# delldu/TransMVSNet

Hardware: AMD Instinct MI355X
Metric: depth maps/sec @ DTU 864x1152 N=5 (48/32/8 hyp); Abs depth L1 vs ref (higher is better)
Workload: dtype f32; 1 GPU; DTU 864x1152, N=5 views, cascade 48/32/8, B=1, hot path from FeatureNet outputs (FMT+pathway+stage glue+cost volume+CostRegNet+softmax/WTA); global_batch=1, parallelism=replica1, launch=hip_graph replay

## Files before the change

### transmvsnet_amd/csrc/costreg.hip

```cpp
#include "common.h"

namespace tmvs {

typedef float floatx4 __attribute__((ext_vector_type(4)));

template <int N>
struct VecN;
template <>
struct VecN<4> {
  float v[4];
  __device__ __forceinline__ void load(const float* p) {
    const float4 t = *reinterpret_cast<const float4*>(p);
    v[0] = t.x;
    v[1] = t.y;
    v[2] = t.z;
    v[3] = t.w;
  }
  __device__ __forceinline__ void zero() { v[0] = v[1] = v[2] = v[3] = 0.f; }
};
template <>
struct VecN<2> {
  float v[2];
  __device__ __forceinline__ void load(const float* p) {
    const float2 t = *reinterpret_cast<const float2*>(p);
// ... 360 lines not shown
            for (int r = 0; r < NBW; ++r)
#pragma unroll
              for (int m = 0; m < MBW; ++m)
                acc[r][m] = __builtin_amdgcn_mfma_f32_16x16x4f32(a[m].v[j], b[r].v[j], acc[r][m], 0, 0, 0);
        }
      }
    }
  }
  if (ow >= g.Wo) return;
  const size_t out_n = (size_t)n * g.Do * g.Ho * g.Wo;
#pragma unroll
  for (int m = 0; m < MBW; ++m) {
    const int co = (mg * MBW + m) * 16 + kgrp * 4;
    if (co >= COUT) continue;
    const float4 al = *reinterpret_cast<const float4*>(alpha + co);
    const float4 sh = *reinterpret_cast<const float4*>(shift + co);
#pragma unroll
    for (int r = 0; r < NBW; ++r) {
      const int oh = hg * NBW + r;
      if (oh >= g.Ho) continue;
      float4 o;
      o.x = act(fmaf(acc[r][m][0], al.x, sh.x), g.lo);
      o.y = act(fmaf(acc[r][m][1], al.y, sh.y), g.lo);
      o.z = act(fmaf(acc[r][m][2], al.z, sh.z), g.lo);
      o.w = act(fmaf(acc[r][m][3], al.w, sh.w), g.lo);
      *reinterpret_cast<float4*>(y + (out_n + ((size_t)od * g.Ho + oh) * g.Wo + ow) * COUT + co) = o;
    }
  }
}

#ifndef TMVS_DECONV_ABL
#define TMVS_DECONV_ABL 0
#endif
template <int CIN, int COUT, int TDI, int THI, int MBB>
__global__ __launch_bounds__(256) void deconv3d_lds_kernel(const float* __restrict__ x,
                                                           const float* __restrict__ wpk,
                                                           const float* __restrict__ alpha,
                                                           const float* __restrict__ shift,
                                                           const float* __restrict__ skip, float* __restrict__ y,
                                                           Geo g) {
  constexpr int CK = CIN < 16 ? CIN : 16;
  constexpr int PL = CK / 4;
  constexpr int MB = (COUT + 15) / 16;
  constexpr int MG = MB / MBB;
  constexpr int NBW = TDI * THI / 4;
  constexpr int LW = 17, LH = THI + 1, LD = TDI + 1;
  constexpr bool SWZ = (CK == 16);
  constexpr int VST = SWZ ? 16 : CK + 4;
  constexpr int NVOX = LD * LH * LW;
  static_assert(MB % MBB == 0 && (TDI * THI) % 4 == 0, "tile");
  static_assert(CK == 16 && MBB == 1, "LDS weight staging assumes 16-channel chunks, one 16-row block");
  constexpr int RM = COUT < 16 ? COUT : 16;
  __shared__ __attribute__((aligned(16))) float tile[NVOX * VST];
  __shared__ __attribute__((aligned(16))) float wts[27 * RM * 16];

  const int nws = (g.Wi + 15) / 16, nhs = (g.Hi + THI - 1) / THI, nds = (g.Di + TDI - 1) / TDI;
  int t = xcd_remap(blockIdx.x, gridDim.x);
  const int mg = t % MG;
  t /= MG;
  const int ws = t % nws;
  t /= nws;
  const int hs = t % nhs;
  t /= nhs;
  const int ds = t % nds;
  const int n = t / nds;
  const int mw0 = ws * 16, mh0 = hs * THI, md0 = ds * TDI;
  const int lane = threadIdx.x & 63, wv = threadIdx.x >> 6;
  const int col = lane & 15, kgrp = lane >> 4;
  const size_t in_n = (size_t)n * g.Di * g.Hi * g.Wi;

  floatx4 acc[NBW][8][MBB];
#pragma unroll
  for (int r = 0; r < NBW; ++r)
#pragma unroll
    for (int c = 0; c < 8; ++c)
#pragma unroll
      for (int m = 0; m < MBB; ++m) acc[r][c][m] = floatx4{0.f, 0.f, 0.f, 0.f};

#pragma unroll 1
  for (int ch = 0; ch < CIN / CK; ++ch) {
    if (ch) __syncthreads();
    for (int idx = threadIdx.x; idx < ((TMVS_DECONV_ABL & 2) ? 0 : NVOX * PL); idx += 256) {
      const int vox = idx / PL, q = idx - vox * PL;
      const int lw = vox % LW, rest = vox / LW, lh = rest % LH, ld = rest / LH;
      const int iw = mw0 + lw, ih = mh0 + lh, id = md0 + ld;
      float4 v = make_float4(0.f, 0.f, 0.f, 0.f);
      if (iw < g.Wi && ih < g.Hi && id < g.Di)
        v = *reinterpret_cast<const float4*>(x + (in_n + ((size_t)id * g.Hi + ih) * g.Wi + iw) * CIN + ch * CK + 4 * q);
      const int qs = SWZ ? (q ^ ((vox >> 1) & 3)) : q;
      *reinterpret_cast<float4*>(tile + vox * VST + 4 * qs) = v;
    }
    for (int idx = threadIdx.x; idx < ((TMVS_DECONV_ABL & 1) ? 0 : 27 * RM * 4); idx += 256) {
      const int q = idx & 3, row = (idx >> 2) % RM, tap = (idx >> 2) / RM;
      const float4 v = *reinterpret_cast<const float4*>(wpk + ((size_t)tap * COUT + mg * 16 + row) * CIN + ch * CK + 4 * q);
      *reinterpret_cast<float4*>(wts + (tap * RM + row) * 16 + 4 * (q ^ ((row >> 1) & 3))) = v;
    }
    __syncthreads();
#pragma unroll
    for (int cls = 0; cls < 8; ++cls) {
      const int pd = cls >> 2, ph = (cls >> 1) & 1, pw = cls & 1;
#pragma unroll
      for (int td = 0; td < 1 + pd; ++td)
#pragma unroll
        for (int th = 0; th < 1 + ph; ++th)
#pragma unroll
          for (int tw = 0; tw < 1 + pw; ++tw) {
            const int kd = pd ? (td ? 2 : 0) : 1, od_off = (pd && !td) ? 1 : 0;
            const int kh = ph ? (th ? 2 : 0) : 1, oh_off = (ph && !th) ? 1 : 0;
            const int kw = pw ? (tw ? 2 : 0) : 1, ow_off = (pw && !tw) ? 1 : 0;
            const int tap = kd * 9 + kh * 3 + kw;
            VecN<PL> a[MBB];
            if (col < RM)
              a[0].load(wts + (tap * RM + col) * 16 + 4 * (kgrp ^ ((col >> 1) & 3)));
            else
              a[0].zero();
#pragma unroll
            for (int r = 0; r < NBW; ++r) {
              const int rr = wv * NBW + r;
              const int mdl = rr / THI, mhl = rr - mdl * THI;
              VecN<PL> b;
              const int lvox = ((mdl + od_off) * LH + mhl + oh_off) * LW + col + ow_off;
              const int qs = SWZ ? (kgrp ^ ((lvox >> 1) & 3)) : kgrp;
              b.load(tile + lvox * VST + qs * PL);
#pragma unroll
              for (int j = 0; j < PL; ++j)
#pragma unroll
                for (int m = 0; m < MBB; ++m) {
                  if (TMVS_DECONV_ABL & 4)
                    acc[r][cls][m][0] = fmaf(a[m].v[j], b.v[j], acc[r][cls][m][0]);
                  else
                    acc[r][cls][m] = __builtin_amdgcn_mfma_f32_16x16x4f32(a[m].v[j], b.v[j], acc[r][cls][m], 0, 0, 0);
                }
            }
          }
    }
  }
  const size_t out_n = (size_t)n * g.Do * g.Ho * g.Wo;
  if constexpr (COUT == 8) {
    __shared__ __attribute__((aligned(16))) float ep[4][32 * 8];
    float* eb = ep[wv];
    const int co = kgrp * 4;
    float4 al = make_float4(0.f, 0.f, 0.f, 0.f), sh = al;
    if (kgrp < 2) {
// ... 29 lines not shown
    }
    return;
  }
  const int mw = mw0 + col;
  if (mw >= g.Wi) return;
#pragma unroll
  for (int m = 0; m < MBB; ++m) {
    const int co = (mg * MBB + m) * 16 + kgrp * 4;
    if (co >= COUT) continue;
    const float4 al = *reinterpret_cast<const float4*>(alpha + co);
    const float4 sh = *reinterpret_cast<const float4*>(shift + co);
#pragma unroll
    for (int r = 0; r < NBW; ++r) {
      const int rr = wv * NBW + r;
      const int md = md0 + rr / THI, mh = mh0 + rr % THI;
      if (md >= g.Di || mh >= g.Hi) continue;
#pragma unroll
      for (int cls = 0; cls < 8; ++cls) {
        const int od = 2 * md + (cls >> 2), oh = 2 * mh + ((cls >> 1) & 1), ow = 2 * mw + (cls & 1);
        const size_t o = (out_n + ((size_t)od * g.Ho + oh) * g.Wo + ow) * COUT + co;
        const float4 s = skip ? *reinterpret_cast<const float4*>(skip + o) : make_float4(0.f, 0.f, 0.f, 0.f);
        float4 v;
        v.x = s.x + act(fmaf(acc[r][cls][m][0], al.x, sh.x), g.lo);
        v.y = s.y + act(fmaf(acc[r][cls][m][1], al.y, sh.y), g.lo);
        v.z = s.z + act(fmaf(acc[r][cls][m][2], al.z, sh.z), g.lo);
        v.w = s.w + act(fmaf(acc[r][cls][m][3], al.w, sh.w), g.lo);
        *reinterpret_cast<float4*>(y + o) = v;
      }
    }
  }
}

constexpr int kDChunk = 8;

constexpr int kProbCols = 62;
typedef float float2_v __attribute__((ext_vector_type(2)));

__device__ __forceinline__ float lane_from_left(float v) {
  return __int_as_float(__builtin_amdgcn_update_dpp(0, __float_as_int(v), 0x138, 0xF, 0xF, false));
}
__device__ __forceinline__ float lane_from_right(float v) {
  return __int_as_float(__builtin_amdgcn_update_dpp(0, __float_as_int(v), 0x130, 0xF, 0xF, false));
}

__global__ __launch_bounds__(256) void conv0_kernel(const float* __restrict__ x, float* __restrict__ y, int D, int H,
                                                    int W, const float* __restrict__ wt,
                                                    const float* __restrict__ alpha,
                                                    const float* __restrict__ shift, float lo) {
  const int HW = H * W;
  const int nseg = (W + kProbCols - 1) / kProbCols, nrow = (H + 3) / 4, ndc = (D + kDChunk - 1) / kDChunk;
  int lb = xcd_remap(blockIdx.x, gridDim.x);
  const int seg = lb % nseg;
  lb /= nseg;
  const int rowb = lb % nrow;
  lb /= nrow;
  const int dc = lb % ndc;
  const int n = lb / ndc;
  const int lane = threadIdx.x & 63;
  const int h = rowb * 4 + (threadIdx.x >> 6);
  if (h >= H) return;
  const int w = seg * kProbCols + lane - 1;
  const bool writes = lane >= 1 && lane <= kProbCols && w < W;
  const int d0 = dc * kDChunk, d1 = min(D, d0 + kDChunk);
  const __amdgpu_buffer_rsrc_t rx = raw_rsrc(x + (size_t)n * D * HW, (unsigned)(D * HW * 4));
  float* yp = y + ((size_t)n * D * HW + (size_t)h * W + w) * 8;
  const unsigned offw = (unsigned)w < (unsigned)W ? (unsigned)w * 4u : kOffOut;
  unsigned offh[3];
#pragma unroll
  for (int k = 0; k < 3; ++k) offh[k] = (unsigned)(h - 1 + k) < (unsigned)H ? (unsigned)((h - 1 + k) * W) * 4u : kOffOut;
  auto load_raw = [&](int d, float (&o)[3]) {
    const unsigned offd = (unsigned)d < (unsigned)D ? (unsigned)d * (unsigned)HW * 4u : kOffOut;
#pragma unroll
    for (int kh = 0; kh < 3; ++kh) {
      const unsigned off = offd | offh[kh] | offw;
      o[kh] = buf_load_f32(rx, (offd + offh[kh] + offw) | (off & kOffOut));
    }
  };
  auto expand = [&](const float (&r)[3], float (&o)[3][3]) {
#pragma unroll
    for (int kh = 0; kh < 3; ++kh) {
      o[kh][0] = lane_from_left(r[kh]);
      o[kh][1] = r[kh];
      o[kh][2] = lane_from_right(r[kh]);
    }
  };
  float al[8], sh[8];
#pragma unroll
  for (int c = 0; c < 8; ++c) {
    al[c] = alpha[c];
    sh[c] = shift[c];
  }
  float win[3][3][3];
  auto step = [&](int d, float (&raw)[3]) {
    expand(raw, win[2]);
    load_raw(d + 2, raw);
    const float* wk = wt;
// ... 27 lines not shown
  };
  float ra[3];
  load_raw(d0 - 1, ra);
  expand(ra, win[0]);
  load_raw(d0, ra);
  expand(ra, win[1]);
  load_raw(d0 + 1, ra);
  for (int d = d0; d < d1; ++d) step(d, ra);
}


#ifndef TMVS_PROB1_UNIFORM
#define TMVS_PROB1_UNIFORM 1
#endif
template <typename Emit>
__device__ __forceinline__ void prob_walk(__amdgpu_buffer_rsrc_t rx, int w, int h, int D, int H, int W, int d0,
                                          const float* __restrict__ wt, Emit emit) {
  const unsigned offw = (unsigned)w < (unsigned)W ? (unsigned)w * 32u : kOffOut;
  auto load_plane = [&](int i, float4 (&o)[3][2]) {
#pragma unroll
    for (int kh = 0; kh < 3; ++kh) {
      const int ih = h - 1 + kh;
      const unsigned offr = ((unsigned)i < (unsigned)D && (unsigned)ih < (unsigned)H)
                                ? ((unsigned)i * (unsigned)H + (unsigned)ih) * (unsigned)W * 32u
                                : kOffOut;
      const unsigned off = (offr + offw) | ((offr | offw) & kOffOut);
      const floatx4 u = buf_load_f32x4(rx, off);
      const floatx4 v = buf_load_f32x4(rx, off + 16u);
      o[kh][0] = make_float4(u[0], u[1], u[2], u[3]);
      o[kh][1] = make_float4(v[0], v[1], v[2], v[3]);
    }
  };
  float2_v c12 = {0.f, 0.f};
  auto plane = [&](int i, const float4 (&p)[3][2]) {
    float acc_next = 0.f;
#pragma unroll
    for (int kh = 0; kh < 3; ++kh) {
      const float xc[8] = {p[kh][0].x, p[kh][0].y, p[kh][0].z, p[kh][0].w,
                           p[kh][1].x, p[kh][1].y, p[kh][1].z, p[kh][1].w};
      int wo = kh * 72;
      asm volatile("" : "+s"(wo));
      const float* wk = wt + __builtin_amdgcn_readfirstlane(wo);
#pragma unroll
      for (int kw = 0; kw < 3; ++kw) {
#pragma unroll
        for (int c = 0; c < 8; ++c) {
          const float xv = kw == 0 ? lane_from_left(xc[c]) : kw == 1 ? xc[c] : lane_from_right(xc[c]);
          const float2_v wp = *reinterpret_cast<const float2_v*>(wk + 2 * (kw * 8 + c));
          acc_next = fmaf(wk[48 + kw * 8 + c], xv, acc_next);
          c12 = __builtin_elementwise_fma(wp, float2_v{xv, xv}, c12);
        }
      }
      asm volatile("" : "+v"(acc_next), "+v"(c12));
    }
    if (i - 1 >= d0) emit(i - 1, c12.y);
    c12 = float2_v{acc_next, c12.x};
  };
  float4 pa[3][2], pb[3][2];
#if TMVS_PROB1_UNIFORM
  d0 = __builtin_amdgcn_readfirstlane(d0);
#endif
  load_plane(d0 - 1, pa);
#if TMVS_PROB1_UNIFORM
#pragma unroll
  for (int j = 0; j < kDChunk + 2; j += 2) {
    const int i = d0 - 1 + j;
#else
#pragma unroll 1
  for (int i = d0 - 1; i < d0 + kDChunk + 1; i += 2) {
#endif
    load_plane(i + 1, pb);
    plane(i, pa);
    load_plane(i + 2, pa);
    plane(i + 1, pb);
  }
}

#ifndef TMVS_PROB_UNIFORM
#define TMVS_PROB_UNIFORM 2
#endif
template <int NR, typename Emit>
__device__ __forceinline__ void prob_walk_rows(__amdgpu_buffer_rsrc_t rx, int w, int h, int D, int H, int W, int d0,
                                               const float* __restrict__ wt, Emit emit) {
  constexpr int NL = NR + 2;
#if TMVS_PROB_UNIFORM
  d0 = __builtin_amdgcn_readfirstlane(d0);
#endif
  const unsigned offw = (unsigned)w < (unsigned)W ? (unsigned)w * 32u : kOffOut;
  auto load_plane = [&](int i, float4 (&o)[NL][2]) {
#pragma unroll
    for (int j = 0; j < NL; ++j) {
      const int ih = h - 1 + j;
      const unsigned offr = ((unsigned)i < (unsigned)D && (unsigned)ih < (unsigned)H)
                                ? ((unsigned)i * (unsigned)H + (unsigned)ih) * (unsigned)W * 32u
                                : kOffOut;
      const unsigned off = (offr + offw) | ((offr | offw) & kOffOut);
      const floatx4 u = buf_load_f32x4(rx, off);
      const floatx4 v = buf_load_f32x4(rx, off + 16u);
      o[j][0] = make_float4(u[0], u[1], u[2], u[3]);
      o[j][1] = make_float4(v[0], v[1], v[2], v[3]);
    }
  };
  float2_v c12[NR];
#pragma unroll
  for (int r = 0; r < NR; ++r) c12[r] = float2_v{0.f, 0.f};
  auto plane = [&](int i, const float4 (&p)[NL][2]) {
    float acc_next[NR];
#pragma unroll
    for (int r = 0; r < NR; ++r) acc_next[r] = 0.f;
#pragma unroll
    for (int kh = 0; kh < 3; ++kh) {
      int wo = kh * 72;
      asm volatile("" : "+s"(wo));
      const float* wk = wt + __builtin_amdgcn_readfirstlane(wo);
#pragma unroll
      for (int r = 0; r < NR; ++r) {
        const int j = r + kh;
        const float xc[8] = {p[j][0].x, p[j][0].y, p[j][0].z, p[j][0].w, p[j][1].x, p[j][1].y, p[j][1].z, p[j][1].w};
#pragma unroll
        for (int kw = 0; kw < 3; ++kw) {
#pragma unroll
          for (int c = 0; c < 8; ++c) {
            const float xv = kw == 0 ? lane_from_left(xc[c]) : kw == 1 ? xc[c] : lane_from_right(xc[c]);
            const float2_v wp = *reinterpret_cast<const float2_v*>(wk + 2 * (kw * 8 + c));
            acc_next[r] = fmaf(wk[48 + kw * 8 + c], xv, acc_next[r]);
            c12[r] = __builtin_elementwise_fma(wp, float2_v{xv, xv}, c12[r]);
          }
        }
        asm volatile("" : "+v"(acc_next[r]), "+v"(c12[r]));
      }
    }
#pragma unroll
    for (int r = 0; r < NR; ++r) {
      if (i - 1 >= d0) emit(r, i - 1, c12[r].y);
      c12[r] = float2_v{acc_next[r], c12[r].x};
    }
  };
  float4 pa[NL][2], pb[NL][2];
  load_plane(d0 - 1, pa);
#if TMVS_PROB_UNIFORM >= 2
#pragma unroll
  for (int j = 0; j < kDChunk + 2; j += 2) {
    const int i = d0 - 1 + j;
#else
#pragma unroll 1
  for (int i = d0 - 1; i < d0 + kDChunk + 1; i += 2) {
#endif
    load_plane(i + 1, pb);
    plane(i, pa);
    load_plane(i + 2, pa);
    plane(i + 1, pb);
  }
}

#ifndef TMVS_PROB_ROWS
#define TMVS_PROB_ROWS 1
#endif
#ifndef TMVS_PROB_WTA_ROWS
#define TMVS_PROB_WTA_ROWS 2
#endif

template <int NR>
__global__ __launch_bounds__(256) void prob_rows_kernel(const float* __restrict__ x, float* __restrict__ y, int D, int H,
                                                        int W, const float* __restrict__ wt) {
  const int HW = H * W;
  const int nseg = (W + kProbCols - 1) / kProbCols, nrow = (H + 4 * NR - 1) / (4 * NR), ndc = (D + kDChunk - 1) / kDChunk;
  int lb = xcd_remap(blockIdx.x, gridDim.x);
  const int seg = lb % nseg;
  lb /= nseg;
  const int rowb = lb % nrow;
  lb /= nrow;
  const int dc = lb % ndc;
  const int n = lb / ndc;
  const int lane = threadIdx.x & 63;
  const int h = (rowb * 4 + (threadIdx.x >> 6)) * NR;
  if (h >= H) return;
  const int w = seg * kProbCols + lane - 1;
  const bool writes = lane >= 1 && lane <= kProbCols && w < W;
  const int d0 = dc * kDChunk, d1 = min(D, d0 + kDChunk);
  const __amdgpu_buffer_rsrc_t rx = raw_rsrc(x + (size_t)n * D * HW * 8, (unsigned)(D * HW * 32));
  float* yn = y + (size_t)n * D * HW + (size_t)h * W + w;
  prob_walk_rows<NR>(rx, w, h, D, H, W, d0, wt, [&](int r, int d, float v) {
    if (d < d1 && writes && h + r < H) yn[(size_t)d * HW + (size_t)r * W] = v;
  });
}
// ... 66 lines not shown
    const float* __restrict__ x, const float* __restrict__ wt, const float* __restrict__ hyp, int H, int W, float lo,
    float hi, float* __restrict__ prob, float* __restrict__ depth, float* __restrict__ depth_raw,
    float* __restrict__ conf) {
  __shared__ float lg[D * 64];
  const int HW = H * W;
  const int nseg = (W + kProbCols - 1) / kProbCols;
  int lb = xcd_remap(blockIdx.x, gridDim.x);
  const int seg = lb % nseg;
  lb /= nseg;
  const int h = lb % H;
  const int n = lb / H;
  const int lane = threadIdx.x & 63;
  const int d0 = (threadIdx.x >> 6) * kDChunk;
  const int w = seg * kProbCols + lane - 1;
  const bool writes = lane >= 1 && lane <= kProbCols && w < W;
  const __amdgpu_buffer_rsrc_t rx = raw_rsrc(x + (size_t)n * D * HW * 8, (unsigned)(D * HW * 32));
  prob_walk(rx, w, h, D, H, W, d0, wt, [&](int d, float v) { lg[d * 64 + lane] = v; });
  __syncthreads();
  if (threadIdx.x >= 64 || !writes) return;
  float xl[D];
#pragma unroll
  for (int d = 0; d < D; ++d) xl[d] = lg[d * 64 + lane];
  const size_t base = (size_t)n * D * HW + (size_t)h * W + w;
  float best;
  const int bi = softmax_first_max<D>(xl, [&](int d, float pr) { prob[base + (size_t)d * HW] = pr; }, best);
  const size_t o = (size_t)n * HW + (size_t)h * W + w;
  const float dr = hyp[base + (size_t)bi * HW];
  depth_raw[o] = dr;
  depth[o] = fminf(fmaxf(dr, lo), hi);
  conf[o] = best;
}


template <int TD, int TH, int NWV = 4>
__global__ __launch_bounds__(NWV * 64) __attribute__((amdgpu_waves_per_eu(NWV == 8 ? 4 : 2))) void conv3d_c16_kernel(const float* __restrict__ x, const float* __restrict__ wpk,
                                                         const float* __restrict__ alpha,
                                                         const float* __restrict__ shift, float* __restrict__ y, Geo g,
                                                         int ntiles) {
  constexpr int C = 16, PL = 4, NBW = TD * TH / NWV, NTH = NWV * 64;
  static_assert(TD * TH % NWV == 0, "rows split evenly over the waves");
  constexpr int LW = 18, LH = TH + 2, LD = TD + 2, VST = 16;
  constexpr int NVOX = LD * LH * LW;
  constexpr int NLD = (NVOX * 4 + NTH - 1) / NTH;
  __shared__ __attribute__((aligned(16))) float tile[NVOX * VST];
  __shared__ __attribute__((aligned(16))) float wts[27 * 16 * 16];
  const int nws = (g.Wo + 15) / 16, nhs = (g.Ho + TH - 1) / TH, nds = (g.Do + TD - 1) / TD;
  const int lane = threadIdx.x & 63, wv = threadIdx.x >> 6;
  const int col = lane & 15, kgrp = lane >> 4;
  const int nxcd = gridDim.x >= 8 ? 8 : 1, per_xcd = gridDim.x / nxcd;
  const int xcd = blockIdx.x % nxcd, kx = blockIdx.x / nxcd;
  const int t_lo = (int)((long)ntiles * xcd / nxcd), t_hi = (int)((long)ntiles * (xcd + 1) / nxcd);
  if (kx >= per_xcd) return;
  struct TileCoord {
    int n, od0, oh0, ow0;
  };
  auto coord = [&](int t) {
    TileCoord c;
    c.ow0 = (t % nws) * 16;
    t /= nws;
    c.oh0 = (t % nhs) * TH;
    t /= nhs;
    c.od0 = (t % nds) * TD;
    c.n = t / nds;
    return c;
  };
  float4 pf[NLD];
  auto fetch = [&](int t) {
    const TileCoord c = coord(t);
    const size_t in_n = (size_t)c.n * g.Di * g.Hi * g.Wi;
#pragma unroll
    for (int k = 0; k < NLD; ++k) {
      const int idx = threadIdx.x + NTH * k;
      const int vox = idx >> 2, q = idx & 3;
      const int lw = vox % LW, rest = vox / LW, lh = rest % LH, ld = rest / LH;
      const int iw = c.ow0 - 1 + lw, ih = c.oh0 - 1 + lh, id = c.od0 - 1 + ld;
      pf[k] = make_float4(0.f, 0.f, 0.f, 0.f);
      if (vox < NVOX && (unsigned)iw < (unsigned)g.Wi && (unsigned)ih < (unsigned)g.Hi && (unsigned)id < (unsigned)g.Di)
        pf[k] = *reinterpret_cast<const float4*>(x + (in_n + ((size_t)id * g.Hi + ih) * g.Wi + iw) * C + 4 * q);
    }
  };
  auto commit = [&]() {
#pragma unroll
    for (int k = 0; k < NLD; ++k) {
      const int idx = threadIdx.x + NTH * k;
      const int vox = idx >> 2, q = idx & 3;
      if (vox < NVOX) *reinterpret_cast<float4*>(tile + vox * VST + 4 * (q ^ ((vox >> 1) & 3))) = pf[k];
    }
  };
  for (int idx = threadIdx.x; idx < 27 * 16 * 4; idx += NTH) {
    const int q = idx & 3, row = (idx >> 2) & 15, tap = idx >> 6;
    const float4 v = *reinterpret_cast<const float4*>(wpk + ((size_t)tap * C + row) * C + 4 * q);
    *reinterpret_cast<float4*>(wts + (tap * 16 + row) * 16 + 4 * (q ^ ((row >> 1) & 3))) = v;
  }
  const float4 al = *reinterpret_cast<const float4*>(alpha + kgrp * 4);
  const float4 sh = *reinterpret_cast<const float4*>(shift + kgrp * 4);
  int t = t_lo + kx;
  if (t < t_hi) {
    fetch(t);
    commit();
  }
  __syncthreads();
  for (; t < t_hi; t += per_xcd) {
    const TileCoord c = coord(t);
    const int tn = t + per_xcd;
    if (tn < t_hi) fetch(tn);
    floatx4 acc[NBW];
#pragma unroll
    for (int r = 0; r < NBW; ++r) acc[r] = floatx4{0.f, 0.f, 0.f, 0.f};
#pragma unroll
    for (int tap = 0; tap < 27; ++tap) {
      const int kd = tap / 9, kh = (tap / 3) % 3, kw = tap % 3;
      VecN<PL> a;
      a.load(wts + (tap * 16 + col) * 16 + 4 * (kgrp ^ ((col >> 1) & 3)));
      VecN<PL> b[NBW];
#pragma unroll
      for (int r = 0; r < NBW; ++r) {
        const int rr = wv * NBW + r;
        const int odl = rr / TH, ohl = rr - odl * TH;
        const int lvox = ((odl + kd) * LH + ohl + kh) * LW + col + kw;
        b[r].load(tile + lvox * VST + 4 * (kgrp ^ ((lvox >> 1) & 3)));
      }
#pragma unroll
      for (int j = 0; j < PL; ++j)
#pragma unroll
        for (int r = 0; r < NBW; ++r)
          acc[r] = __builtin_amdgcn_mfma_f32_16x16x4f32(a.v[j], b[r].v[j], acc[r], 0, 0, 0);
      if (tap % (NBW > 2 ? 3 : 9) == (NBW > 2 ? 2 : 8)) __builtin_amdgcn_sched_barrier(0);
    }
    const int ow = c.ow0 + col;
    const size_t out_n = (size_t)c.n * g.Do * g.Ho * g.Wo;
#pragma unroll
    for (int r = 0; r < NBW; ++r) {
      const int rr = wv * NBW + r;
      const int od = c.od0 + rr / TH, oh = c.oh0 + rr % TH;
      if (ow >= g.Wo || od >= g.Do || oh >= g.Ho) continue;
      float4 o;
      o.x = act(fmaf(acc[r][0], al.x, sh.x), g.lo);
      o.y = act(fmaf(acc[r][1], al.y, sh.y), g.lo);
      o.z = act(fmaf(acc[r][2], al.z, sh.z), g.lo);
      o.w = act(fmaf(acc[r][3], al.w, sh.w), g.lo);
      *reinterpret_cast<float4*>(y + (out_n + ((size_t)od * g.Ho + oh) * g.Wo + ow) * C + kgrp * 4) = o;
    }
    __syncthreads();
    if (tn < t_hi) commit();
    __syncthreads();
  }
}

template <typename K>
static int persistent_grid(K kernel, long ntiles, int block = 256) {
  struct Entry {
    const void* fn;
    int dev, cap;
  };
  static Entry cache[16];
  static int used = 0;
  int dev = 0;
  hipGetDevice(&dev);
  for (int i = 0; i < used; ++i)
    if (cache[i].fn == (const void*)kernel && cache[i].dev == dev) return (int)std::min<long>(ntiles, cache[i].cap);
  int cus = 0, per = 0;
  hipDeviceGetAttribute(&cus, hipDeviceAttributeMultiprocessorCount, dev);
  hipOccupancyMaxActiveBlocksPerMultiprocessor(&per, kernel, block, 0);
  const int cap = std::max(8, cus * std::max(per, 1));
  if (used < 16) cache[used++] = Entry{(const void*)kernel, dev, cap};
  return (int)std::min<long>(ntiles, cap);
}

#ifndef TMVS_C16_NWV
#define TMVS_C16_NWV 4
#endif
template <int TD, int TH>
static int launch_conv_c16(const float* x, const float* w, const float* al, const float* sh, float* y, int B,
                           const Geo& g, hipStream_t st) {
  constexpr int NWV = TMVS_C16_NWV;
  const long ntiles = (long)B * ((g.Do + TD - 1) / TD) * ((g.Ho + TH - 1) / TH) * ((g.Wo + 15) / 16);
  const int grid = persistent_grid(conv3d_c16_kernel<TD, TH, NWV>, ntiles, NWV * 64);
  hipLaunchKernelGGL((conv3d_c16_kernel<TD, TH, NWV>), dim3(grid), dim3(NWV * 64), 0, st, x, w, al, sh, y, g,
                     (int)ntiles);
  TMVS_CHECK_LAUNCH();
  return TMVS_OK;
}

template <int TD, int TH, int NWV = 4>
__global__ __launch_bounds__(NWV * 64) __attribute__((amdgpu_waves_per_eu(NWV == 8 ? 4 : 1))) void conv3d_s2c8_tile_kernel(const float* __restrict__ x,
                                                               const float* __restrict__ wpk,
                                                               const float* __restrict__ alpha,
                                                               const float* __restrict__ shift, float* __restrict__ y,
                                                               Geo g, int ntiles) {
  constexpr int CIN = 8, COUT = 16, NBW = TD * TH / NWV, NTH = NWV * 64;
  static_assert(TD * TH % NWV == 0, "rows split evenly over the waves");
  constexpr int LW = 33, LH = 2 * TH + 1, LD = 2 * TD + 1, SW = 17;
  constexpr int NROW = LD * LH, NQ = NROW * LW * 2;
  constexpr int NLD = (NQ + NTH - 1) / NTH;
  __shared__ __attribute__((aligned(16))) float tile[NROW * 2 * SW * 8];
  __shared__ __attribute__((aligned(16))) float wts[28 * 16 * 8];
  const int nws = (g.Wo + 15) / 16, nhs = (g.Ho + TH - 1) / TH, nds = (g.Do + TD - 1) / TD;
  const int lane = threadIdx.x & 63, wv = threadIdx.x >> 6;
  const int col = lane & 15, kgrp = lane >> 4;
  const int half = kgrp & 1, side = kgrp >> 1;
  const int nxcd = gridDim.x >= 8 ? 8 : 1, per_xcd = gridDim.x / nxcd;
  const int xcd = blockIdx.x % nxcd, kx = blockIdx.x / nxcd;
  const int t_lo = (int)((long)ntiles * xcd / nxcd), t_hi = (int)((long)ntiles * (xcd + 1) / nxcd);
  if (kx >= per_xcd) return;
  struct TileCoord {
    int n, od0, oh0, ow0;
  };
  auto coord = [&](int t) {
    TileCoord c;
    c.ow0 = (t % nws) * 16;
    t /= nws;
    c.oh0 = (t % nhs) * TH;
// ... 290 lines not shown
    }
#pragma unroll
    for (int r = 0; r < NBW; ++r)
#pragma unroll
      for (int pdh = 0; pdh < 4; ++pdh) {
        const floatx4 a = acc[r][pdh];
        *reinterpret_cast<float4*>(eb + (2 * col + (kgrp >> 1)) * 8 + cq) =
            make_float4(act(fmaf(a[0], al.x, sh.x), g.lo), act(fmaf(a[1], al.y, sh.y), g.lo), act(fmaf(a[2], al.z, sh.z), g.lo),
                        act(fmaf(a[3], al.w, sh.w), g.lo));
        __builtin_amdgcn_wave_barrier();
        const float4 v = *reinterpret_cast<const float4*>(eb + lane * 4);
        __builtin_amdgcn_wave_barrier();
        const float4 sv = sk[r][pdh];
        if (ok[r])
          *reinterpret_cast<float4*>(y + oo[r] + (pdh >> 1) * plane + (pdh & 1) * row) =
              make_float4(sv.x + v.x, sv.y + v.y, sv.z + v.z, sv.w + v.w);
      }
    if (tn < t_hi) commit(tile[(it + 1) & 1]);
    __syncthreads();
  }
}

template <int TDI, int THI>
static int launch_deconv_c8(const float* x, const float* w, const float* al, const float* sh, const float* skip,
                            float* y, int B, const Geo& g, hipStream_t st) {
  const long ntiles = (long)B * ((g.Di + TDI - 1) / TDI) * ((g.Hi + THI - 1) / THI) * ((g.Wi + 15) / 16);
  const long grid = persistent_grid(deconv3d_c8_kernel<TDI, THI>, ntiles);
  hipLaunchKernelGGL((deconv3d_c8_kernel<TDI, THI>), dim3((unsigned)grid), dim3(256), 0, st, x, w, al, sh, skip, y, g,
                     (int)ntiles);
  TMVS_CHECK_LAUNCH();
  return TMVS_OK;
}

template <int CIN, int COUT, int TDI, int THI, int MBB>
static int launch_deconv(const float* x, const float* w, const float* al, const float* sh, const float* skip,
                         float* y, int B, const Geo& g, hipStream_t st) {
  constexpr int MG = ((COUT + 15) / 16) / MBB;
  const long nblk = (long)B * ((g.Di + TDI - 1) / TDI) * ((g.Hi + THI - 1) / THI) * ((g.Wi + 15) / 16) * MG;
  hipLaunchKernelGGL((deconv3d_lds_kernel<CIN, COUT, TDI, THI, MBB>), dim3((unsigned)nblk), dim3(256), 0, st, x, w,
                     al, sh, skip, y, g);
  TMVS_CHECK_LAUNCH();
  return TMVS_OK;
}

static int conv_dispatch(const float* x, int B, int cin, int d, int h, int w, const float* wpk, const float* al,
                         const float* sh, int cout, int stride, float* y, hipStream_t st, float lo = 0.f) {
  Geo g;
  g.lo = lo;
  g.Di = d;
  g.Hi = h;
  g.Wi = w;
  if (stride == 1) {
    g.Do = d;
    g.Ho = h;
    g.Wo = w;
  } else {
    g.Do = (d - 1) / 2 + 1;
    g.Ho = (h - 1) / 2 + 1;
    g.Wo = (w - 1) / 2 + 1;
  }
  if ((long long)d * h * w * cin * 4 >= (1LL << 31)) return TMVS_ERR_SHAPE;
#define TMVS_CONV_LDS(CI, CO, ...)                                                              \
  if (cin == CI && cout == CO && stride == 1) {                                               \
    return launch_conv<CI, CO, 1, __VA_ARGS__>(x, wpk, al, sh, y, B, g, st);                 \
  }
#ifndef TMVS_C16_TD
#define TMVS_C16_TD 2
#define TMVS_C16_TH 4
#endif
#ifdef TMVS_C16_LDS
  TMVS_CONV_LDS(16, 16, TMVS_C16_LDS)
#endif
  if (cin == 16 && cout == 16 && stride == 1)
// ... 30 lines not shown
#define TMVS_CONV_DIRECT(CI, CO, NBW, MBW) \
  if (cin == CI && cout == CO && stride == 2) return launch_conv_direct<CI, CO, 2, NBW, MBW>(x, wpk, al, sh, y, B, g, st);
  TMVS_CONV_DIRECT(8, 16, 4, 1)
  TMVS_CONV_DIRECT(16, 32, 4, 1)
#ifndef TMVS_C5_LDS
#define TMVS_C5_LDS 1, 2, 4, 4
#endif
#ifndef TMVS_C5_MODE
#define TMVS_C5_MODE 2
#endif
  if (cin == 32 && cout == 64 && stride == 2) {
    if constexpr (TMVS_C5_MODE == 2) return launch_conv_tapout<32, 64, 2, TMVS_C5_LDS>(x, wpk, al, sh, y, B, g, st);
    if constexpr (TMVS_C5_MODE == 1) return launch_conv<32, 64, 2, TMVS_C5_LDS>(x, wpk, al, sh, y, B, g, st);
  }
  TMVS_CONV_DIRECT(32, 64, 2, 1)
#undef TMVS_CONV_DIRECT
  return TMVS_ERR_SHAPE;
}

static int deconv_dispatch(const float* x, int B, int cin, int d, int h, int w, const float* wpk, const float* al,
                           const float* sh, int cout, const float* skip, float* y, hipStream_t st, float lo = 0.f) {
  Geo g;
  g.lo = lo;
  g.Di = d;
  g.Hi = h;
  g.Wi = w;
  g.Do = 2 * d;
  g.Ho = 2 * h;
  g.Wo = 2 * w;
#ifndef TMVS_DECONV_EVEN
#define TMVS_DECONV_EVEN 2, 2
#define TMVS_DECONV_ODD 1, 4
#endif
#define TMVS_DECONV_CASE(CI, CO, MBB)                                                                       \
  if (cin == CI && cout == CO) {                                                                           \
    if (g.Di % 2 == 0) return launch_deconv<CI, CO, TMVS_DECONV_EVEN, MBB>(x, wpk, al, sh, skip, y, B, g, st); \
    return launch_deconv<CI, CO, TMVS_DECONV_ODD, MBB>(x, wpk, al, sh, skip, y, B, g, st);                  \
  }
  TMVS_DECONV_CASE(64, 32, 1)
  TMVS_DECONV_CASE(32, 16, 1)
  if (cin == 16 && cout == 8) {
    if (g.Di % 2 == 0) return launch_deconv_c8<2, 2>(x, wpk, al, sh, skip, y, B, g, st);
    return launch_deconv_c8<1, 4>(x, wpk, al, sh, skip, y, B, g, st);
  }
#undef TMVS_DECONV_CASE
  return TMVS_ERR_SHAPE;
}

}

using namespace tmvs;

extern "C" int tmvs_conv3d_bn_relu(const float* x, int batch, int cin, int d, int h, int w, const float* wpk,
                                   const float* alpha, const float* shift, int cout, int stride, float* y,
                                   void* stream) {
  if (!x || !wpk || !alpha || !shift || !y || batch <= 0 || d <= 0 || h <= 0 || w <= 0) return TMVS_ERR_ARG;
  if (stride != 1 && stride != 2) return TMVS_ERR_ARG;
  return conv_dispatch(x, batch, cin, d, h, w, wpk, alpha, shift, cout, stride, y, (hipStream_t)stream);
}

extern "C" int tmvs_deconv3d_bn_relu_add(const float* x, int batch, int cin, int d, int h, int w, const float* wpk,
                                         const float* alpha, const float* shift, int cout, const float* skip,
                                         float* y, void* stream) {
  if (!x || !wpk || !alpha || !shift || !skip || !y || batch <= 0 || d <= 0 || h <= 0 || w <= 0)
    return TMVS_ERR_ARG;
  return deconv_dispatch(x, batch, cin, d, h, w, wpk, alpha, shift, cout, skip, y, (hipStream_t)stream);
}

// ... 11 lines not shown
    hipLaunchKernelGGL(prob_kernel, prob_grid(batch, D, H, W, kDChunk), dim3(256), 0, st, x, y, D, H, W, wt);
  }
  TMVS_CHECK_LAUNCH();
  return TMVS_OK;
}

__device__ float kUnitAlpha[64] = {1.f, 1.f, 1.f, 1.f, 1.f, 1.f, 1.f, 1.f, 1.f, 1.f, 1.f, 1.f, 1.f, 1.f, 1.f, 1.f,
                                   1.f, 1.f, 1.f, 1.f, 1.f, 1.f, 1.f, 1.f, 1.f, 1.f, 1.f, 1.f, 1.f, 1.f, 1.f, 1.f,
                                   1.f, 1.f, 1.f, 1.f, 1.f, 1.f, 1.f, 1.f, 1.f, 1.f, 1.f, 1.f, 1.f, 1.f, 1.f, 1.f,
                                   1.f, 1.f, 1.f, 1.f, 1.f, 1.f, 1.f, 1.f, 1.f, 1.f, 1.f, 1.f, 1.f, 1.f, 1.f, 1.f};
__device__ float kZeroShift[64];

extern "C" int tmvs_conv3d_mfma(const float* x, int batch, int cin, int d, int h, int w, const float* wpk, int cout,
                                int stride, int transposed, const float* skip, float* y, void* stream) {
  if (!x || !wpk || !y || batch <= 0 || d <= 0 || h <= 0 || w <= 0) return TMVS_ERR_ARG;
  if (transposed ? stride != 2 : (stride != 1 && stride != 2)) return TMVS_ERR_ARG;
  if (skip && !transposed) return TMVS_ERR_ARG;
  int dev = 0;
  if (hipGetDevice(&dev) != hipSuccess || dev < 0 || dev >= 64) return TMVS_ERR_HIP;
  static const float* unit[64][2];
  if (!unit[dev][0]) {
    void *a, *b;
    if (hipGetSymbolAddress(&a, HIP_SYMBOL(kUnitAlpha)) != hipSuccess ||
        hipGetSymbolAddress(&b, HIP_SYMBOL(kZeroShift)) != hipSuccess)
      return TMVS_ERR_HIP;
    unit[dev][1] = (const float*)b;
    unit[dev][0] = (const float*)a;
  }
  const float *al = unit[dev][0], *sh = unit[dev][1];
  const float lo = -__builtin_huge_valf();
  hipStream_t st = (hipStream_t)stream;
  if (!transposed && stride == 1 && cin == 1 && cout == 8) {
    if ((long long)d * h * w * 32 >= (1LL << 31)) return TMVS_ERR_SHAPE;
    const dim3 grid((unsigned)(((w + kProbCols - 1) / kProbCols) * ((h + 3) / 4) * batch * ((d + kDChunk - 1) / kDChunk)));
    hipLaunchKernelGGL(conv0_kernel, grid, dim3(256), 0, st, x, y, d, h, w, wpk, al, sh, lo);
    TMVS_CHECK_LAUNCH();
    return TMVS_OK;
  }
  if (!transposed && stride == 1 && cin == 8 && cout == 1) {
    if ((long long)d * h * w * 32 >= (1LL << 31)) return TMVS_ERR_SHAPE;
    return launch_prob(x, y, batch, d, h, w, wpk, st);
  }
  if (transposed) return deconv_dispatch(x, batch, cin, d, h, w, wpk, al, sh, cout, skip, y, st, lo);
  return conv_dispatch(x, batch, cin, d, h, w, wpk, al, sh, cout, stride, y, st, lo);
}

static size_t align_up(size_t v) { return (v + 255) & ~(size_t)255; }

extern "C" size_t tmvs_costregnet_workspace(int batch, int depth, int height, int width, int base_ch) {
  const size_t v0 = (size_t)batch * depth * height * width;
  const size_t v1 = v0 / 8, v2 = v0 / 64, v3 = v0 / 512;
  const size_t c = (size_t)base_ch;
  size_t bytes = 0;
  bytes += align_up(v0 * c * 4);
  bytes += align_up(v1 * 2 * c * 4) * 2;
  bytes += align_up(v2 * 4 * c * 4) * 2;
  bytes += align_up(v3 * 8 * c * 4) * 2;
  bytes += align_up(v2 * 4 * c * 4);
  bytes += align_up(v1 * 2 * c * 4);
  bytes += align_up(v0 * c * 4);
  return bytes;
}

static int costregnet_trunk(const float* x, int batch, int depth, int height, int width, const TmvsCostRegWeights* w,
                            void* workspace, size_t workspace_bytes, hipStream_t st, float** x11_out,
                            float** c0_out) {
  if (!x || !w || !workspace || batch <= 0) return TMVS_ERR_ARG;
  if (depth % 8 || height % 8 || width % 8) return TMVS_ERR_SHAPE;
  if (w->base_ch != 8) return TMVS_ERR_SHAPE;
  if ((long long)depth * height * width * 32 >= (1LL << 31)) return TMVS_ERR_SHAPE;
  for (int i = 0; i < 11; ++i)
    if (!w->w[i]) return TMVS_ERR_ARG;
  for (int i = 0; i < 10; ++i)
    if (!w->alpha[i] || !w->shift[i]) return TMVS_ERR_ARG;
  if (workspace_bytes < tmvs_costregnet_workspace(batch, depth, height, width, w->base_ch)) return TMVS_ERR_ARG;
  const int c = w->base_ch;
  const size_t v0 = (size_t)batch * depth * height * width;
  const size_t v1 = v0 / 8, v2 = v0 / 64, v3 = v0 / 512;
  char* ws = (char*)workspace;
  auto take = [&](size_t n) {
    float* p = (float*)ws;
    ws += align_up(n * 4);
    return p;
  };
  float* c0 = take(v0 * c);
  float* c1 = take(v1 * 2 * c);
  float* c2 = take(v1 * 2 * c);
  float* c3 = take(v2 * 4 * c);
  float* c4 = take(v2 * 4 * c);
  float* c5 = take(v3 * 8 * c);
  float* c6 = take(v3 * 8 * c);
  float* x7 = take(v2 * 4 * c);
  float* x9 = take(v1 * 2 * c);
  float* x11 = take(v0 * c);
  const int D0 = depth, H0 = height, W0 = width;
  const int D1 = D0 / 2, H1 = H0 / 2, W1 = W0 / 2;
  const int D2 = D1 / 2, H2 = H1 / 2, W2 = W1 / 2;
  const int D3 = D2 / 2, H3 = H2 / 2, W3 = W2 / 2;
  int rc;
  const dim3 g0x((unsigned)(((W0 + kProbCols - 1) / kProbCols) * ((H0 + 3) / 4) * batch * ((D0 + kDChunk - 1) / kDChunk)));
  hipLaunchKernelGGL(conv0_kernel, g0x, dim3(256), 0, st, x, c0, D0, H0, W0, w->w[0], w->alpha[0], w->shift[0],
                     0.f);
  TMVS_CHECK_LAUNCH();
  if ((rc = conv_dispatch(c0, batch, c, D0, H0, W0, w->w[1], w->alpha[1], w->shift[1], 2 * c, 2, c1, st))) return rc;
  if ((rc = conv_dispatch(c1, batch, 2 * c, D1, H1, W1, w->w[2], w->alpha[2], w->shift[2], 2 * c, 1, c2, st)))
    return rc;
  if ((rc = conv_dispatch(c2, batch, 2 * c, D1, H1, W1, w->w[3], w->alpha[3], w->shift[3], 4 * c, 2, c3, st)))
    return rc;
  if ((rc = conv_dispatch(c3, batch, 4 * c, D2, H2, W2, w->w[4], w->alpha[4], w->shift[4], 4 * c, 1, c4, st)))
    return rc;
  if ((rc = conv_dispatch(c4, batch, 4 * c, D2, H2, W2, w->w[5], w->alpha[5], w->shift[5], 8 * c, 2, c5, st)))
    return rc;
  if ((rc = conv_dispatch(c5, batch, 8 * c, D3, H3, W3, w->w[6], w->alpha[6], w->shift[6], 8 * c, 1, c6, st)))
    return rc;
  if ((rc = deconv_dispatch(c6, batch, 8 * c, D3, H3, W3, w->w[7], w->alpha[7], w->shift[7], 4 * c, c4, x7, st)))
    return rc;
  if ((rc = deconv_dispatch(x7, batch, 4 * c, D2, H2, W2, w->w[8], w->alpha[8], w->shift[8], 2 * c, c2, x9, st)))
    return rc;
  if ((rc = deconv_dispatch(x9, batch, 2 * c, D1, H1, W1, w->w[9], w->alpha[9], w->shift[9], c, c0, x11, st)))
    return rc;
  *x11_out = x11;
  *c0_out = c0;
  return TMVS_OK;
}

extern "C" int tmvs_costregnet(const float* x, int batch, int depth, int height, int width,
                               const TmvsCostRegWeights* w, void* workspace, size_t workspace_bytes, float* logits,
                               void* stream) {
  if (!logits) return TMVS_ERR_ARG;
  hipStream_t st = (hipStream_t)stream;
  float *x11, *c0;
  int rc;
  if ((rc = costregnet_trunk(x, batch, depth, height, width, w, workspace, workspace_bytes, st, &x11, &c0))) return rc;
// ... 44 lines not shown
```

Measured before the change: 298.7 depth_maps/s.

## Skip zero-padded depth taps at volume edges in conv, deconv and prob kernels

Adds EDGE variants of the 16-channel conv and the LDS deconv kernels. They statically drop MFMA taps that read the zero-padded planes before the first or past the last depth plane, and the conv variant is chosen when the depth extent spans at most two tiles. The uniform prob-head path gets a peeled prologue and epilogue so the first and last chunks skip partial-sum work for out-of-range neighbours. The conv0 depth chunk becomes configurable. This targets the shallow depth levels of the cascade (8 hypotheses and its downsampled levels), where padding taps are a large share of the work, at the cost of more template instantiations and a different row-to-wave mapping.

Result: no change. 301.3 depth_maps/s, median of 6 (+0.9%).

```diff
diff --git a/transmvsnet_amd/csrc/costreg.hip b/transmvsnet_amd/csrc/costreg.hip
--- a/transmvsnet_amd/csrc/costreg.hip
+++ b/transmvsnet_amd/csrc/costreg.hip
@@ -416,7 +416,7 @@
 #ifndef TMVS_DECONV_ABL
 #define TMVS_DECONV_ABL 0
 #endif
-template <int CIN, int COUT, int TDI, int THI, int MBB>
+template <int CIN, int COUT, int TDI, int THI, int MBB, bool EDGE = false>
 __global__ __launch_bounds__(256) void deconv3d_lds_kernel(const float* __restrict__ x,
                                                            const float* __restrict__ wpk,
                                                            const float* __restrict__ alpha,
@@ -434,6 +434,7 @@
   constexpr int NVOX = LD * LH * LW;
   static_assert(MB % MBB == 0 && (TDI * THI) % 4 == 0, "tile");
   static_assert(CK == 16 && MBB == 1, "LDS weight staging assumes 16-channel chunks, one 16-row block");
+  static_assert(!EDGE || TDI == 1, "EDGE: one input plane per tile");
   constexpr int RM = COUT < 16 ? COUT : 16;
   __shared__ __attribute__((aligned(16))) float tile[NVOX * VST];
   __shared__ __attribute__((aligned(16))) float wts[27 * RM * 16];
@@ -493,6 +494,7 @@
             const int kh = ph ? (th ? 2 : 0) : 1, oh_off = (ph && !th) ? 1 : 0;
             const int kw = pw ? (tw ? 2 : 0) : 1, ow_off = (pw && !tw) ? 1 : 0;
             const int tap = kd * 9 + kh * 3 + kw;
+            if (EDGE && od_off) continue;
             VecN<PL> a[MBB];
             if (col < RM)
               a[0].load(wts + (tap * RM + col) * 16 + 4 * (kgrp ^ ((col >> 1) & 3)));
@@ -588,6 +590,10 @@
 }
 
 constexpr int kDChunk = 8;
+#ifndef TMVS_CONV0_DCHUNK
+#define TMVS_CONV0_DCHUNK 8
+#endif
+constexpr int kConv0Chunk = TMVS_CONV0_DCHUNK;
 
 constexpr int kProbCols = 62;
 typedef float float2_v __attribute__((ext_vector_type(2)));
@@ -604,7 +610,7 @@
                                                     const float* __restrict__ alpha,
                                                     const float* __restrict__ shift, float lo) {
   const int HW = H * W;
-  const int nseg = (W + kProbCols - 1) / kProbCols, nrow = (H + 3) / 4, ndc = (D + kDChunk - 1) / kDChunk;
+  const int nseg = (W + kProbCols - 1) / kProbCols, nrow = (H + 3) / 4, ndc = (D + kConv0Chunk - 1) / kConv0Chunk;
   int lb = xcd_remap(blockIdx.x, gridDim.x);
   const int seg = lb % nseg;
   lb /= nseg;
@@ -617,7 +623,7 @@
   if (h >= H) return;
   const int w = seg * kProbCols + lane - 1;
   const bool writes = lane >= 1 && lane <= kProbCols && w < W;
-  const int d0 = dc * kDChunk, d1 = min(D, d0 + kDChunk);
+  const int d0 = dc * kConv0Chunk, d1 = min(D, d0 + kConv0Chunk);
   const __amdgpu_buffer_rsrc_t rx = raw_rsrc(x + (size_t)n * D * HW, (unsigned)(D * HW * 4));
   float* yp = y + ((size_t)n * D * HW + (size_t)h * W + w) * 8;
   const unsigned offw = (unsigned)w < (unsigned)W ? (unsigned)w * 4u : kOffOut;
@@ -711,7 +717,8 @@
     }
   };
   float2_v c12 = {0.f, 0.f};
-  auto plane = [&](int i, const float4 (&p)[3][2]) {
+  auto plane = [&](auto which, int i, const float4 (&p)[3][2]) {
+    constexpr int WHICH = decltype(which)::value;
     float acc_next = 0.f;
 #pragma unroll
     for (int kh = 0; kh < 3; ++kh) {
@@ -725,9 +732,12 @@
 #pragma unroll
         for (int c = 0; c < 8; ++c) {
           const float xv = kw == 0 ? lane_from_left(xc[c]) : kw == 1 ? xc[c] : lane_from_right(xc[c]);
-          const float2_v wp = *reinterpret_cast<const float2_v*>(wk + 2 * (kw * 8 + c));
-          acc_next = fmaf(wk[48 + kw * 8 + c], xv, acc_next);
-          c12 = __builtin_elementwise_fma(wp, float2_v{xv, xv}, c12);
+          if constexpr (WHICH == 0 || WHICH == 1) acc_next = fmaf(wk[48 + kw * 8 + c], xv, acc_next);
+          if constexpr (WHICH == 0 || WHICH == 2) {
+            const float2_v wp = *reinterpret_cast<const float2_v*>(wk + 2 * (kw * 8 + c));
+            c12 = __builtin_elementwise_fma(wp, float2_v{xv, xv}, c12);
+          }
+          if constexpr (WHICH == 3) c12.y = fmaf(wk[2 * (kw * 8 + c) + 1], xv, c12.y);
         }
       }
       asm volatile("" : "+v"(acc_next), "+v"(c12));
@@ -735,24 +745,43 @@
     if (i - 1 >= d0) emit(i - 1, c12.y);
     c12 = float2_v{acc_next, c12.x};
   };
+  using All = std::integral_constant<int, 0>;
+  using NextOnly = std::integral_constant<int, 1>;
+  using NoNext = std::integral_constant<int, 2>;
+  using LastOnly = std::integral_constant<int, 3>;
   float4 pa[3][2], pb[3][2];
 #if TMVS_PROB1_UNIFORM
   d0 = __builtin_amdgcn_readfirstlane(d0);
-#endif
+  const bool front = d0 > 0, back = d0 + kDChunk < D;
+  if (front) load_plane(d0 - 1, pa);
+  load_plane(d0, pb);
+  if (front) plane(NextOnly{}, d0 - 1, pa);
+#pragma unroll
+  for (int j = 0; j < kDChunk - 2; j += 2) {
+    const int i = d0 + j;
+    load_plane(i + 1, pa);
+    plane(All{}, i, pb);
+    load_plane(i + 2, pb);
+    plane(All{}, i + 1, pa);
+  }
+  load_plane(d0 + kDChunk - 1, pa);
+  plane(All{}, d0 + kDChunk - 2, pb);
+  load_plane(d0 + kDChunk, pb);
+  plane(NoNext{}, d0 + kDChunk - 1, pa);
+  if (back)
+    plane(LastOnly{}, d0 + kDChunk, pb);
+  else
+    emit(d0 + kDChunk - 1, c12.y);
+#else
   load_plane(d0 - 1, pa);
-#if TMVS_PROB1_UNIFORM
-#pragma unroll
-  for (int j = 0; j < kDChunk + 2; j += 2) {
-    const int i = d0 - 1 + j;
-#else
 #pragma unroll 1
   for (int i = d0 - 1; i < d0 + kDChunk + 1; i += 2) {
-#endif
     load_plane(i + 1, pb);
-    plane(i, pa);
+    plane(All{}, i, pa);
     load_plane(i + 2, pa);
-    plane(i + 1, pb);
-  }
+    plane(All{}, i + 1, pb);
+  }
+#endif
 }
 
 #ifndef TMVS_PROB_UNIFORM
@@ -783,7 +812,8 @@
   float2_v c12[NR];
 #pragma unroll
   for (int r = 0; r < NR; ++r) c12[r] = float2_v{0.f, 0.f};
-  auto plane = [&](int i, const float4 (&p)[NL][2]) {
+  auto plane = [&](auto which, int i, const float4 (&p)[NL][2]) {
+    constexpr int WHICH = decltype(which)::value;
     float acc_next[NR];
 #pragma unroll
     for (int r = 0; r < NR; ++r) acc_next[r] = 0.f;
@@ -801,9 +831,12 @@
 #pragma unroll
           for (int c = 0; c < 8; ++c) {
             const float xv = kw == 0 ? lane_from_left(xc[c]) : kw == 1 ? xc[c] : lane_from_right(xc[c]);
-            const float2_v wp = *reinterpret_cast<const float2_v*>(wk + 2 * (kw * 8 + c));
-            acc_next[r] = fmaf(wk[48 + kw * 8 + c], xv, acc_next[r]);
-            c12[r] = __builtin_elementwise_fma(wp, float2_v{xv, xv}, c12[r]);
+            if constexpr (WHICH == 0 || WHICH == 1) acc_next[r] = fmaf(wk[48 + kw * 8 + c], xv, acc_next[r]);
+            if constexpr (WHICH == 0 || WHICH == 2) {
+              const float2_v wp = *reinterpret_cast<const float2_v*>(wk + 2 * (kw * 8 + c));
+              c12[r] = __builtin_elementwise_fma(wp, float2_v{xv, xv}, c12[r]);
+            }
+            if constexpr (WHICH == 3) c12[r].y = fmaf(wk[2 * (kw * 8 + c) + 1], xv, c12[r].y);
           }
         }
         asm volatile("" : "+v"(acc_next[r]), "+v"(c12[r]));
@@ -815,21 +848,44 @@
       c12[r] = float2_v{acc_next[r], c12[r].x};
     }
   };
+  using All = std::integral_constant<int, 0>;
+  using NextOnly = std::integral_constant<int, 1>;
+  using NoNext = std::integral_constant<int, 2>;
+  using LastOnly = std::integral_constant<int, 3>;
   float4 pa[NL][2], pb[NL][2];
+#if TMVS_PROB_UNIFORM >= 2
+  const bool front = d0 > 0, back = d0 + kDChunk < D;
+  if (front) load_plane(d0 - 1, pa);
+  load_plane(d0, pb);
+  if (front) plane(NextOnly{}, d0 - 1, pa);
+#pragma unroll
+  for (int j = 0; j < kDChunk - 2; j += 2) {
+    const int i = d0 + j;
+    load_plane(i + 1, pa);
+    plane(All{}, i, pb);
+    load_plane(i + 2, pb);
+    plane(All{}, i + 1, pa);
+  }
+  load_plane(d0 + kDChunk - 1, pa);
+  plane(All{}, d0 + kDChunk - 2, pb);
+  if (back) load_plane(d0 + kDChunk, pb);
+  plane(NoNext{}, d0 + kDChunk - 1, pa);
+  if (back) {
+    plane(LastOnly{}, d0 + kDChunk, pb);
+  } else {
+#pragma unroll
+    for (int r = 0; r < NR; ++r) emit(r, d0 + kDChunk - 1, c12[r].y);
+  }
+#else
   load_plane(d0 - 1, pa);
-#if TMVS_PROB_UNIFORM >= 2
-#pragma unroll
-  for (int j = 0; j < kDChunk + 2; j += 2) {
-    const int i = d0 - 1 + j;
-#else
 #pragma unroll 1
   for (int i = d0 - 1; i < d0 + kDChunk + 1; i += 2) {
-#endif
     load_plane(i + 1, pb);
-    plane(i, pa);
+    plane(All{}, i, pa);
     load_plane(i + 2, pa);
-    plane(i + 1, pb);
-  }
+    plane(All{}, i + 1, pb);
+  }
+#endif
 }
 
 #ifndef TMVS_PROB_ROWS
@@ -962,13 +1018,14 @@
 }
 
 
-template <int TD, int TH, int NWV = 4>
+template <int TD, int TH, int NWV = 4, bool EDGE = false>
 __global__ __launch_bounds__(NWV * 64) __attribute__((amdgpu_waves_per_eu(NWV == 8 ? 4 : 2))) void conv3d_c16_kernel(const float* __restrict__ x, const float* __restrict__ wpk,
                                                          const float* __restrict__ alpha,
                                                          const float* __restrict__ shift, float* __restrict__ y, Geo g,
                                                          int ntiles) {
   constexpr int C = 16, PL = 4, NBW = TD * TH / NWV, NTH = NWV * 64;
   static_assert(TD * TH % NWV == 0, "rows split evenly over the waves");
+  static_assert(!EDGE || NBW % TD == 0, "EDGE deals every wave the same number of rows of each plane");
   constexpr int LW = 18, LH = TH + 2, LD = TD + 2, VST = 16;
   constexpr int NVOX = LD * LH * LW;
   constexpr int NLD = (NVOX * 4 + NTH - 1) / NTH;
@@ -1030,6 +1087,8 @@
     commit();
   }
   __syncthreads();
+  auto row_od = [&](int r) { return EDGE ? r % TD : (wv * NBW + r) / TH; };
+  auto row_oh = [&](int r) { return EDGE ? wv * (NBW / TD) + r / TD : (wv * NBW + r) % TH; };
   for (; t < t_hi; t += per_xcd) {
     const TileCoord c = coord(t);
     const int tn = t + per_xcd;
@@ -1037,32 +1096,49 @@
     floatx4 acc[NBW];
 #pragma unroll
     for (int r = 0; r < NBW; ++r) acc[r] = floatx4{0.f, 0.f, 0.f, 0.f};
-#pragma unroll
-    for (int tap = 0; tap < 27; ++tap) {
-      const int kd = tap / 9, kh = (tap / 3) % 3, kw = tap % 3;
-      VecN<PL> a;
-      a.load(wts + (tap * 16 + col) * 16 + 4 * (kgrp ^ ((col >> 1) & 3)));
-      VecN<PL> b[NBW];
-#pragma unroll
-      for (int r = 0; r < NBW; ++r) {
-        const int rr = wv * NBW + r;
-        const int odl = rr / TH, ohl = rr - odl * TH;
-        const int lvox = ((odl + kd) * LH + ohl + kh) * LW + col + kw;
-        b[r].load(tile + lvox * VST + 4 * (kgrp ^ ((lvox >> 1) & 3)));
+    auto taps = [&](auto front, auto back) {
+      constexpr bool FRONT = decltype(front)::value, BACK = decltype(back)::value;
+#pragma unroll
+      for (int tap = 0; tap < 27; ++tap) {
+        const int kd = tap / 9, kh = (tap / 3) % 3, kw = tap % 3;
+        VecN<PL> a;
+        a.load(wts + (tap * 16 + col) * 16 + 4 * (kgrp ^ ((col >> 1) & 3)));
+        VecN<PL> b[NBW];
+        bool skip[NBW];
+#pragma unroll
+        for (int r = 0; r < NBW; ++r) {
+          skip[r] = EDGE && ((FRONT && kd == 0 && r % TD == 0) || (BACK && kd == 2 && r % TD == TD - 1));
+          if (skip[r]) continue;
+          const int odl = row_od(r), ohl = row_oh(r);
+          const int lvox = ((odl + kd) * LH + ohl + kh) * LW + col + kw;
+          b[r].load(tile + lvox * VST + 4 * (kgrp ^ ((lvox >> 1) & 3)));
+        }
+#pragma unroll
+        for (int j = 0; j < PL; ++j)
+#pragma unroll
+          for (int r = 0; r < NBW; ++r)
+            if (!skip[r]) acc[r] = __builtin_amdgcn_mfma_f32_16x16x4f32(a.v[j], b[r].v[j], acc[r], 0, 0, 0);
+        if (tap % (NBW > 2 ? 3 : 9) == (NBW > 2 ? 2 : 8)) __builtin_amdgcn_sched_barrier(0);
       }
-#pragma unroll
-      for (int j = 0; j < PL; ++j)
-#pragma unroll
-        for (int r = 0; r < NBW; ++r)
-          acc[r] = __builtin_amdgcn_mfma_f32_16x16x4f32(a.v[j], b[r].v[j], acc[r], 0, 0, 0);
-      if (tap % (NBW > 2 ? 3 : 9) == (NBW > 2 ? 2 : 8)) __builtin_amdgcn_sched_barrier(0);
+    };
+    if constexpr (EDGE) {
+      const bool fr = c.od0 == 0, bk = c.od0 + TD >= g.Di;
+      if (fr && bk)
+        taps(std::true_type{}, std::true_type{});
+      else if (fr)
+        taps(std::true_type{}, std::false_type{});
+      else if (bk)
+        taps(std::false_type{}, std::true_type{});
+      else
+        taps(std::false_type{}, std::false_type{});
+    } else {
+      taps(std::false_type{}, std::false_type{});
     }
     const int ow = c.ow0 + col;
     const size_t out_n = (size_t)c.n * g.Do * g.Ho * g.Wo;
 #pragma unroll
     for (int r = 0; r < NBW; ++r) {
-      const int rr = wv * NBW + r;
-      const int od = c.od0 + rr / TH, oh = c.oh0 + rr % TH;
+      const int od = c.od0 + row_od(r), oh = c.oh0 + row_oh(r);
       if (ow >= g.Wo || od >= g.Do || oh >= g.Ho) continue;
       float4 o;
       o.x = act(fmaf(acc[r][0], al.x, sh.x), g.lo);
@@ -1100,14 +1176,23 @@
 #ifndef TMVS_C16_NWV
 #define TMVS_C16_NWV 4
 #endif
+#ifndef TMVS_C16_EDGE_MAX_TILES
+#define TMVS_C16_EDGE_MAX_TILES 2
+#endif
 template <int TD, int TH>
 static int launch_conv_c16(const float* x, const float* w, const float* al, const float* sh, float* y, int B,
                            const Geo& g, hipStream_t st) {
   constexpr int NWV = TMVS_C16_NWV;
   const long ntiles = (long)B * ((g.Do + TD - 1) / TD) * ((g.Ho + TH - 1) / TH) * ((g.Wo + 15) / 16);
-  const int grid = persistent_grid(conv3d_c16_kernel<TD, TH, NWV>, ntiles, NWV * 64);
-  hipLaunchKernelGGL((conv3d_c16_kernel<TD, TH, NWV>), dim3(grid), dim3(NWV * 64), 0, st, x, w, al, sh, y, g,
-                     (int)ntiles);
+  if (g.Do <= TMVS_C16_EDGE_MAX_TILES * TD) {
+    const int grid = persistent_grid(conv3d_c16_kernel<TD, TH, NWV, true>, ntiles, NWV * 64);
+    hipLaunchKernelGGL((conv3d_c16_kernel<TD, TH, NWV, true>), dim3(grid), dim3(NWV * 64), 0, st, x, w, al, sh, y, g,
+                       (int)ntiles);
+  } else {
+    const int grid = persistent_grid(conv3d_c16_kernel<TD, TH, NWV>, ntiles, NWV * 64);
+    hipLaunchKernelGGL((conv3d_c16_kernel<TD, TH, NWV>), dim3(grid), dim3(NWV * 64), 0, st, x, w, al, sh, y, g,
+                       (int)ntiles);
+  }
   TMVS_CHECK_LAUNCH();
   return TMVS_OK;
 }
@@ -1464,13 +1549,13 @@
   return TMVS_OK;
 }
 
-template <int CIN, int COUT, int TDI, int THI, int MBB>
+template <int CIN, int COUT, int TDI, int THI, int MBB, bool EDGE = false>
 static int launch_deconv(const float* x, const float* w, const float* al, const float* sh, const float* skip,
                          float* y, int B, const Geo& g, hipStream_t st) {
   constexpr int MG = ((COUT + 15) / 16) / MBB;
   const long nblk = (long)B * ((g.Di + TDI - 1) / TDI) * ((g.Hi + THI - 1) / THI) * ((g.Wi + 15) / 16) * MG;
-  hipLaunchKernelGGL((deconv3d_lds_kernel<CIN, COUT, TDI, THI, MBB>), dim3((unsigned)nblk), dim3(256), 0, st, x, w,
-                     al, sh, skip, y, g);
+  hipLaunchKernelGGL((deconv3d_lds_kernel<CIN, COUT, TDI, THI, MBB, EDGE>), dim3((unsigned)nblk), dim3(256), 0, st, x,
+                     w, al, sh, skip, y, g);
   TMVS_CHECK_LAUNCH();
   return TMVS_OK;
 }
@@ -1567,8 +1652,13 @@
 #define TMVS_DECONV_EVEN 2, 2
 #define TMVS_DECONV_ODD 1, 4
 #endif
+#ifndef TMVS_DECONV_EDGE
+#define TMVS_DECONV_EDGE 1
+#endif
 #define TMVS_DECONV_CASE(CI, CO, MBB)                                                                       \
   if (cin == CI && cout == CO) {                                                                           \
+    if (g.Di == 1 && TMVS_DECONV_EDGE)                                                                       \
+      return launch_deconv<CI, CO, 1, 4, MBB, true>(x, wpk, al, sh, skip, y, B, g, st);                     \
     if (g.Di % 2 == 0) return launch_deconv<CI, CO, TMVS_DECONV_EVEN, MBB>(x, wpk, al, sh, skip, y, B, g, st); \
     return launch_deconv<CI, CO, TMVS_DECONV_ODD, MBB>(x, wpk, al, sh, skip, y, B, g, st);                  \
   }
@@ -1646,7 +1736,7 @@
   hipStream_t st = (hipStream_t)stream;
   if (!transposed && stride == 1 && cin == 1 && cout == 8) {
     if ((long long)d * h * w * 32 >= (1LL << 31)) return TMVS_ERR_SHAPE;
-    const dim3 grid((unsigned)(((w + kProbCols - 1) / kProbCols) * ((h + 3) / 4) * batch * ((d + kDChunk - 1) / kDChunk)));
+    const dim3 grid((unsigned)(((w + kProbCols - 1) / kProbCols) * ((h + 3) / 4) * batch * ((d + kConv0Chunk - 1) / kConv0Chunk)));
     hipLaunchKernelGGL(conv0_kernel, grid, dim3(256), 0, st, x, y, d, h, w, wpk, al, sh, lo);
     TMVS_CHECK_LAUNCH();
     return TMVS_OK;
@@ -1712,7 +1802,7 @@
   const int D2 = D1 / 2, H2 = H1 / 2, W2 = W1 / 2;
   const int D3 = D2 / 2, H3 = H2 / 2, W3 = W2 / 2;
   int rc;
-  const dim3 g0x((unsigned)(((W0 + kProbCols - 1) / kProbCols) * ((H0 + 3) / 4) * batch * ((D0 + kDChunk - 1) / kDChunk)));
+  const dim3 g0x((unsigned)(((W0 + kProbCols - 1) / kProbCols) * ((H0 + 3) / 4) * batch * ((D0 + kConv0Chunk - 1) / kConv0Chunk)));
   hipLaunchKernelGGL(conv0_kernel, g0x, dim3(256), 0, st, x, c0, D0, H0, W0, w->w[0], w->alpha[0], w->shift[0],
                      0.f);
   TMVS_CHECK_LAUNCH();
```
